# snowzurfer/raytracer-gamma

Measured on AMD Instinct MI355X. Metric: Mpixels/s (primary rays) + frame ms at WxH, depth D; PPM max-abs-diff vs CPU, higher is better.
Workload: dtype f32; 1 GPU; c3: 3840x2160, 16 spheres, 3 lights, depth 5 (RTSTACK_MAXSIZE 6), 3x3 supersampling; width=3840, height=2160, spheres=16, lights=3, depth=5, alias_factor=3, row_block=8, variant=0, parallelism=row-cyclic x1

## Files before the change

### raytracer-gamma_amd/csrc/rtg_scene_pack.h

```cpp
#pragma once

#include <math.h>
#include <string.h>

#include <algorithm>
#include <functional>
#include <thread>
#include <utility>
#include <vector>

#include "rtg.h"
#include "rtg_internal.h"
#include "rtg_trace.h"

namespace rtg {

constexpr unsigned kMaskMaxSpheres = 64;

struct PackedScene {
  std::vector<float> geom, crad2, mats, lights;
  std::vector<float> prim;
  std::vector<unsigned> smask;
  std::vector<unsigned> cone;
  std::vector<float> bvhNodes;
// ... 595 lines not shown
        cr = rc * rc;
        child = ~(int)i;
      } else {
        float mn[3] = {__builtin_inff(), __builtin_inff(), __builtin_inff()};
        float mx[3] = {-__builtin_inff(), -__builtin_inff(), -__builtin_inff()};
        for (unsigned t = a; t < b; ++t)
          for (int q = 0; q < 3; ++q) {
            mn[q] = fminf(mn[q], gb[6 * (size_t)idx[t] + q]);
            mx[q] = fmaxf(mx[q], gb[6 * (size_t)idx[t] + 3 + q]);
          }
        for (int q = 0; q < 3; ++q) {
          s[q] = mn[q];
          s[3 + q] = mx[q];
        }
        child = build(a, b, depth + 1);
      }
      float* rec = &ps->bvhNodes[(size_t)node * kBvhWords];
      for (int q = 0; q < 6; ++q) rec[6 * k + q] = s[q];
      memcpy(&rec[24 + k], &child, 4);
      rec[28 + k] = cr;
    }
    return node;
  };
  build(0, n, 0);
  if (depthOut) *depthOut = maxDepth;
  if (maxDepth > 20) {
    ps->bvhNodes.clear();
    return false;
  }
  if ((double)(ps->bvhNodes.size() / kBvhWords) * kBvhCopies * kBvhWords * 4.0 >= 0x1p32) {
    ps->bvhNodes.clear();
    return false;
  }
  {
    const std::vector<float> src = ps->bvhNodes;
    const size_t nn = src.size() / kBvhWords;
    ps->bvhNodes.assign(nn * 8 * kBvhWords, 0.f);
    for (size_t nd = 0; nd < nn; ++nd) {
      const float* in = &src[nd * kBvhWords];
      for (unsigned oct = 0; oct < 8; ++oct) {
        const double sg[3] = {(oct & 1u) ? -1.0 : 1.0, (oct & 2u) ? -1.0 : 1.0,
                              (oct & 4u) ? -1.0 : 1.0};
        int ord[4] = {0, 1, 2, 3};
        double key[4];
        int cls[4];
        for (int k = 0; k < 4; ++k) {
          int ch;
          memcpy(&ch, &in[24 + k], 4);
          key[k] = 0.0;
          cls[k] = ch > 0 ? 0 : ch < 0 ? 1 : 2;
          if (ch > 0) {
            for (int q = 0; q < 3; ++q) {
              const double lo = in[6 * k + q], hi = in[6 * k + 3 + q];
              key[k] += sg[q] * (sg[q] > 0 ? lo : hi);
            }
          } else if (ch < 0) {
            for (int q = 0; q < 3; ++q) key[k] += sg[q] * (double)in[6 * k + q];
            key[k] = key[k] * 0.5773502691896258 - (double)in[6 * k + 5];
          }
        }
        std::stable_sort(ord, ord + 4, [&](int a, int b) {
          return cls[a] != cls[b] ? cls[a] < cls[b] : key[a] < key[b];
        });
        float* out = &ps->bvhNodes[(nd * 8 + oct) * kBvhWords];
        for (int k = 0; k < 4; ++k) {
          const int j = ord[k];
          for (int q = 0; q < 6; ++q) out[6 * k + q] = in[6 * j + q];
          out[24 + k] = in[24 + j];
          out[28 + k] = in[28 + j];
        }
      }
    }
  }
  return true;
}

inline void pack_scene(const rtg_sphere* spheres, unsigned n, const rtg_light* lights,
                       unsigned m, PackedScene* ps) {
  ps->n = n;
  ps->m = m;
  ps->n4 = (n + 3u) & ~3u;
  ps->geom.assign((size_t)(ps->n4 + 4) * 20, __builtin_nanf(""));
  ps->crad2.assign(n ? 3 * (size_t)n : 1, 0.f);
  ps->mats.assign((size_t)(n + 1) * 8, 0.f);
  ps->lights.assign((size_t)(m ? m : 1) * 6, 0.f);
  ps->prim.assign((size_t)(n ? n : 1) * 4, 0.f);
  for (unsigned i = 0; i < n; ++i) {
    const rtg_sphere& s = spheres[i];
    float* g = &ps->geom[(size_t)i * 4];
    g[0] = s.pos.x; g[1] = s.pos.y; g[2] = s.pos.z;
    g[3] = s.radius * s.radius;
    float* gs = &ps->geom[(size_t)(ps->n4 + 4 + i) * 4];
    gs[0] = g[0]; gs[1] = g[1]; gs[2] = g[2];
    gs[3] = screen_r2(g[3]);
    float* gc = &ps->geom[(size_t)(2 * (ps->n4 + 4) + i) * 4];
    gc[0] = g[0]; gc[1] = g[1]; gc[2] = g[2];
    const float rc = s.radius + 1.0e-6f;
    ps->crad2[i] = rc * rc;
    gc[3] = ps->crad2[i];
    const float dx = 0.f - s.pos.x, dy = 0.f - s.pos.y, dz = 0.f - s.pos.z;
    ps->crad2[n + i] = (((dx * dx) + (dy * dy)) + (dz * dz)) - g[3];
    ps->crad2[2 * (size_t)n + i] = guard_r2(s);
    float* gf = &ps->geom[(size_t)(ps->n4 + 4) * 12 + (size_t)i * 8];
    gf[0] = g[0]; gf[1] = g[1]; gf[2] = g[2];
    gf[3] = gs[3];
    gf[4] = g[3];
    gf[5] = ps->crad2[n + i];
    gf[6] = 0.f; gf[7] = 0.f;
    prim_consts(s, &ps->prim[(size_t)i * 4]);
    float* mt = &ps->mats[(size_t)i * 8];
    mt[0] = s.material.matteColour.x; mt[1] = s.material.matteColour.y;
    mt[2] = s.material.matteColour.z; mt[3] = s.material.glossColour.x;
    mt[4] = s.material.glossColour.y; mt[5] = s.material.glossColour.z;
    mt[6] = s.material.opacity; mt[7] = s.material.refractiveIndex;
  }
  ps->mats[(size_t)n * 8 + 7] = 1.00f;
  shadow_masks(spheres, n, lights, m, &ps->smask);
  if (!ps->smask.empty()) cone_masks(spheres, n, &ps->cone);
  else ps->cone.clear();
  if (build_bvh(spheres, n, ps)) {
    sphere_lists(spheres, n, lights, m, ps);
  }
  for (unsigned l = 0; l < m; ++l) {
    float* p = &ps->lights[(size_t)l * 6];
    p[0] = lights[l].pos.x; p[1] = lights[l].pos.y; p[2] = lights[l].pos.z;
    p[3] = lights[l].col.x; p[4] = lights[l].col.y; p[5] = lights[l].col.z;
  }
}

inline int make_camera(unsigned W, unsigned H, float zoom, float aa, Camera* cam) {
  if (W == 0 || H == 0) {
    rtg_set_error("empty frame %ux%u", W, H);
    return RTG_ERR_INVALID;
  }
  if (!(aa <= 256.f)) {
    rtg_set_error("aliasFactor %g out of range", (double)aa);
    return RTG_ERR_INVALID;
  }
  cam->xs = 16.f / ((float)W);
  cam->ys = 12.f / ((float)H);
  cam->asp = 16.f / 12.f;
  cam->st = cam->xs / aa;
  const float tot = aa * aa;
  cam->inv = 1.f / tot;
  cam->halfW = W * 0.5f;
  cam->halfH = H * 0.5f;
  cam->zoom = zoom;
  int k = 0;
  while ((float)k < aa) ++k;
  cam->nAA = k;
  return RTG_OK;
}

}
```

### raytracer-gamma_amd/csrc/rtg_trace.h

```cpp
#pragma once

#include <string.h>

#include <stdint.h>
#include <math.h>

#include <type_traits>

#if defined(__HIPCC__)
#include <hip/hip_runtime.h>
#define RTG_HD __host__ __device__ __forceinline__
#else
#define RTG_HD inline
#endif

namespace rtg {

struct V3 { float x, y, z; };

RTG_HD V3 v3(float a, float b, float c) { V3 r; r.x = a; r.y = b; r.z = c; return r; }
RTG_HD V3 vadd(V3 a, V3 b) { return v3(a.x + b.x, a.y + b.y, a.z + b.z); }
RTG_HD V3 vsub(V3 a, V3 b) { return v3(a.x - b.x, a.y - b.y, a.z - b.z); }
RTG_HD V3 vmul(V3 a, V3 b) { return v3(a.x * b.x, a.y * b.y, a.z * b.z); }
RTG_HD V3 vsmul(float k, V3 b) { return v3(k * b.x, k * b.y, k * b.z); }
// ... 57 lines not shown
    no_speculate();
    if (!rcp_fast_range(b)) y = 1.f / b;
  }
  return y;
}
RTG_HD float cull_rsq(float x) {
#if defined(__HIP_DEVICE_COMPILE__)
  return __builtin_amdgcn_rsqf(x);
#else
  return 1.0f / sqrtf(x);
#endif
}
RTG_HD float rtg_sqrtf(float x) { return sqrt_rn(x); }
RTG_HD float rcp_sqrt_rn(float x) {
  float y = rcp_fast(sqrt_fast(x));
  if (any_lane(!sqrt_fast_range(x))) {
    no_speculate();
    if (!sqrt_fast_range(x)) y = 1.f / sqrtf(x);
  }
  return y;
}
RTG_HD V3 vnorm(V3 v) { float l = rcp_sqrt_rn(vdot(v, v)); return vsmul(l, v); }
RTG_HD bool significant(V3 c) { return (c.x >= 0.001f) || (c.y >= 0.001f) || (c.z >= 0.001f); }

struct Camera {
  float xs, ys, asp, st, inv, halfW, halfH, zoom;
  int nAA;
};

struct Mat { V3 matte, gloss; float opacity, refr; };

enum : int { kFusePrim = 1, kFuseCone = 2, kFuseShadow = 4, kFuseEnter = 8 };

enum : int { kCntSamples = 0, kCntPrimQ, kCntPrimSel, kCntPrimCand, kCntEnterQ, kCntEnterOK,
             kCntFullQ, kCntFullCand, kCntShadowQ, kCntShadowSel, kCntShadowCand,
             kCntContainMasked, kCntContainSel, kCntContainFull, kCntRefraction, kCntReflPush,
             kCntBvhNodeTests, kCntBvhSphereTests, kCntConeQ, kCntConeSel,
             kCntBvhShadowQ, kCntBvhShadowNodeTests, kCntBvhShadowSphereTests,
             kUQuery,
             kUPrimIter,
             kUPrimExact,
             kUSelIter,
             kUSelExact,
             kUShdIter,
             kUShdExact,
             kUEnterHead,
             kUEnterIter,
             kUEnterExact,
             kUFullGroup,
             kUFullExact,
             kUBvhNode,
             kUBvhSlot,
             kUBvhExact,
             kUContIter,
             kUCont4,
             kUContBvhNode,
             kUCone,
             kUMaskIter,
             kUNode,
             kUShade,
             kULight,
             kUShadow,
             kULit,
             kURefr,
             kURefrLeaf,
             kUPush,
             kUDescend,
             kUUnwind,
             kUSample,
             kUBvhPass,
             kUCapIter,
             kUOvIter,
             kUDiagShdSame,
             kUDiagEnterAll,
             kUDiagEnterSame,
             kUDiagContSame,
             kULightDir,
             kUDiagInsig,
             kUDiagInsigAll,
             kUWave,
             kUQueryHead,
             kUDiagShdEmpty,
             kUDiagConeEmpty,
             kCntSlots };
enum : int { kProbeClosest = 0, kProbeShadow = 1, kProbeRefraction = 2, kProbeTotal = 3,
             kProbeMatte = 4, kProbePush = 5, kProbeUnwind = 6, kProbeShade = 7,
             kProbeSlots = 8 };

struct FrameC {
  float cx, cy, cz;
  unsigned meta;
};
struct FrameR { V3 ro, rd, rI; };

template <int NF>
struct LocalFrames {
  FrameC f[NF];
  RTG_HD FrameC get(int lv) const { return f[lv]; }
  RTG_HD void set(int lv, const FrameC& v) { f[lv] = v; }
};

struct Frame {
  V3 colour;
  V3 ro, rd, rI;
  int rm;
  int flags;
};

struct RayQ {
  V3 o, d;
  float a4, den, y;
  float ap;
  bool fast;
  bool slow;
};

RTG_HD RayQ query_head(V3 o, V3 d, float& a) {
  RayQ q{};
  q.o = o;
  q.d = d;
  a = vdot(d, d);
  q.a4 = 4.0f * a;
  return q;
}
RTG_HD void query_rest(RayQ& q, float a) {
  q.den = 2.0f * a;
  q.ap = a * (1.0f - 0x1p-16f);
  q.fast = (q.den >= 0x1p-60f) && (q.den <= 0x1p60f);
  q.slow = any_lane(!q.fast);
  q.y = rcp_fast(q.den);
}

RTG_HD RayQ make_query(V3 o, V3 d) {
  float a;
  RayQ q = query_head(o, d, a);
  query_rest(q, a);
  return q;
}

RTG_HD float quot(float x, const RayQ& q) {
  const float q0 = x * q.y;
  const float r0 = fmaf(-q0, q.den, x);
  const float q1 = fmaf(r0, q.y, q0);
  const float r1 = fmaf(-q1, q.den, x);
  float r = fmaf(r1, q.y, q1);
  if (q.slow) {
    no_speculate();
    if (!q.fast) r = x / q.den;
  }
  return r;
}

template <bool kFast>
RTG_HD float quot_k(float x, const RayQ& q) {
  if constexpr (kFast) {
    const float q0 = x * q.y;
    const float r0 = fmaf(-q0, q.den, x);
    const float q1 = fmaf(r0, q.y, q0);
    const float r1 = fmaf(-q1, q.den, x);
    return fmaf(r1, q.y, q1);
  } else {
    return quot(x, q);
  }
}

#ifndef RTG_NOROOT_K
// ... 295 lines not shown
            blk = blocked_cap_lanes(sc, P, dir, gap, l, hit, cell, hc, hr2, full);
          }
          if (sc.any(full))
            if (full) blk = query_blocked<2>(sc, P, dir, gap);
        }
      } else {
        blk = query_blocked<Q>(sc, P, dir, gap);
      }
      sc.probe_end(kProbeShadow);
      if (!blk) {
        sc.count(kULit, 1);
        const float intensity = incidence / gap;
        sum = vadd(sum, vsmul(intensity, Lcol));
        if constexpr (RP::kOn) rp.lit(l);
      }
    }
  }
  return sum;
}

RTG_HD double sqrt_d_unit(double y) {
#if defined(__HIP_DEVICE_COMPILE__)
  const double g = __builtin_amdgcn_rsq(y);
  double s = y * g;
  double h = g * 0.5;
  const double r = fma(-h, s, 0.5);
  s = fma(s, r, s);
  h = fma(h, r, h);
  double d = fma(-s, s, y);
  s = fma(d, h, s);
  d = fma(-s, s, y);
  s = fma(d, h, s);
  return y == 0.0 ? 0.0 : s;
#else
  return sqrt(y);
#endif
}
RTG_HD double div_d_fresnel(double a, double b, bool fast) {
#if defined(__HIP_DEVICE_COMPILE__)
  double y = __builtin_amdgcn_rcp(b);
  double e = fma(-b, y, 1.0);
  y = fma(y, e, y);
  e = fma(-b, y, 1.0);
  y = fma(y, e, y);
  const double q = a * y;
  const double r = fma(-b, q, a);
  double d = fma(r, y, q);
  if (any_lane(!fast)) {
    no_speculate();
    if (!fast) d = a / b;
  }
  return d;
#else
  (void)fast;
  return a / b;
#endif
}

template <bool kCL = false>
RTG_HD float polarised_reflection(float n1, float n2, float cosA1, float cosA2) {
  const float left = n1 * cosA1;
  const float right = n2 * cosA2;
  if constexpr (kCL) {
    const float num = left - right;
    float den = left + right;
    den *= den;
    if (den < 1.0e-6f) return 1.f;
    float refl = (num * num) / den;
    if (refl > 1.f) refl = 1.f;
    return refl;
  }
  const double num = (double)(left - right);
  double den = (double)(left + right);
  den *= den;
  const bool tiny = den < (double)1.0e-6f;
  const bool fast = fabsf(left) <= 0x1p100f && fabsf(right) <= 0x1p100f;
  float refl = (float)div_d_fresnel(num * num, den, fast || tiny);
  if (refl > 1.f) refl = 1.f;
  return tiny ? 1.f : refl;
}

template <bool kCL = false, class Scene>
RTG_HD int refraction(const Scene& sc, V3 D, V3 P, V3 N, float nSrc, bool wantRay,
                      V3& dirOut, float& R, int hit = -1, bool guardOK = false) {
  float cosA1 = vdot(D, N);
  float sinA1 = 0.f;
  if (cosA1 <= -1.0f) { cosA1 = -1.f; sinA1 = 0.f; }
  else if (cosA1 >= 1.f) { cosA1 = 1.f; sinA1 = 0.f; }
  else sinA1 = (float)sqrt_d_unit(1.0 - (double)(cosA1 * cosA1));

  const V3 testPt = vadd(vsmul(0.01f, D), P);
  int tgt;
  float nTgt;
  if (hit >= 0 && sc.has_smask()) {
    const bool ok = guardOK && vdot(D, D) <= kContainDirMax * kContainDirMax;
    const uint64_t cu = sc.contain_union(hit, ok);
    sc.count(kCntContainMasked, 1);
    sc.count(kCntContainSel, __builtin_popcountll(cu));
    tgt = primary_container_sel(sc, testPt, cu, nTgt);
    if (tgt < 0) tgt = (int)sc.n;
  } else {
    bool full = true;
    tgt = -1;
    if (hit >= 0 && sc.has_lists() &&
        sc.all(guardOK && vdot(D, D) <= kContainDirMax * kContainDirMax)) {
      if (sc.all(sc.first_lane_i(hit) == hit)) sc.count(kUDiagContSame, 1);
      tgt = container_lanes(sc, testPt, hit, nTgt, full);
    }
    if (sc.any(full)) {
      if (full) {
        sc.count(kCntContainFull, 1);
        tgt = primary_container(sc, testPt);
        nTgt = sc.refr(tgt < 0 ? (int)sc.n : tgt);
      }
    }
    if (tgt < 0) tgt = (int)sc.n;
  }
  const float ratio = nSrc / nTgt;
  const float sinA2 = ratio * sinA1;

  if (wantRay) {
    const float qb = 2.f * cosA1;
    const float qc = 1.f - rcp_rn(ratio * ratio);
    const float rad = (qb * qb) - ((4.f * 1.f) * qc);
    float r0, r1;
    int ns;
    if (fabsf(rad) < 0.001f) {
      r0 = -qb / (2.f * 1.f);
      r1 = 0.f;
      ns = 1;
    } else {
      const float root = rtg_sqrtf(rad);
      const float den = 2.0f * 1.f;
      r0 = (-qb + root) / den;
      r1 = (-qb - root) / den;
      ns = 2;
    }
    float maxAlign = (float)-0.1;
    V3 dir = v3(0.f, 0.f, 0.f);
    {
      V3 cur = vadd(D, vsmul(r0, N));
      float al = vdot(D, cur);
      if (al > maxAlign) { maxAlign = al; dir = cur; }
    }
    if (ns == 2) {
      V3 cur = vadd(D, vsmul(r1, N));
      float al = vdot(D, cur);
      if (al > maxAlign) { maxAlign = al; dir = cur; }
    }
    dirOut = dir;
  }
  float cosA2 = rtg_sqrtf(1.f - (sinA2 * sinA2));
  if (cosA1 < 0.f) cosA2 = -cosA2;
  const float Rs = polarised_reflection<kCL>(nSrc, nTgt, cosA1, cosA2);
  const float Rp = polarised_reflection<kCL>(nSrc, nTgt, cosA2, cosA1);
  R = (Rs + Rp) * 0.5f;
  return tgt;
}

template <bool kNT>
RTG_HD void store_frame_r(FrameR& dst, const FrameR& r) {
#if defined(__HIP_DEVICE_COMPILE__)
  if constexpr (kNT) {
    __builtin_nontemporal_store(r.ro.x, &dst.ro.x);
    __builtin_nontemporal_store(r.ro.y, &dst.ro.y);
    __builtin_nontemporal_store(r.ro.z, &dst.ro.z);
    __builtin_nontemporal_store(r.rd.x, &dst.rd.x);
    __builtin_nontemporal_store(r.rd.y, &dst.rd.y);
    __builtin_nontemporal_store(r.rd.z, &dst.rd.z);
    __builtin_nontemporal_store(r.rI.x, &dst.rI.x);
    __builtin_nontemporal_store(r.rI.y, &dst.rI.y);
    __builtin_nontemporal_store(r.rI.z, &dst.rI.z);
    return;
  }
#endif
  dst = r;
}
template <bool kNT>
RTG_HD FrameR load_frame_r(const FrameR& src) {
#if defined(__HIP_DEVICE_COMPILE__)
  if constexpr (kNT) {
    FrameR r;
    r.ro = v3(__builtin_nontemporal_load(&src.ro.x), __builtin_nontemporal_load(&src.ro.y),
              __builtin_nontemporal_load(&src.ro.z));
    r.rd = v3(__builtin_nontemporal_load(&src.rd.x), __builtin_nontemporal_load(&src.rd.y),
              __builtin_nontemporal_load(&src.rd.z));
    r.rI = v3(__builtin_nontemporal_load(&src.rI.x), __builtin_nontemporal_load(&src.rI.y),
              __builtin_nontemporal_load(&src.rI.z));
    return r;
  }
#endif
  return src;
}

template <int S, int Q, bool kCL = false, class RP = NoRayPath, class Scene, class FStore>
RTG_HD V3 trace_sample(const Scene& sc, V3 dir0, FStore&& fc, bool usePrim = false,
                       uint64_t primSel = ~0ull, V3 o0 = V3{0.f, 0.f, 0.f},
                       const RP& rp = RP()) {
  static_assert(!RP::kOn || Q == 2, "a caller's rays run the Q == 2 shading path");
  constexpr int NF = (S > 1) ? (S - 1) : 1;
  FrameR fr[NF];
  int sp = 0;
  V3 ret = v3(0.f, 0.f, 0.f);
  V3 o = o0, d = dir0, I = v3(1.f, 1.f, 1.f);
  int rm = (int)sc.n;
  int enterH = -1;
  int originH = -1;
  for (;;) {
    float t;
    sc.count(kUNode, 1);
    sc.count(kUDiagInsig, significant(I) ? 0 : 1);
    if (sc.all(!significant(I))) sc.count(kUDiagInsigAll, 1);
    sc.probe_begin(kProbeClosest);
    int hit = -1;
    bool full = false;
    if constexpr (RP::kOn) {
      sc.count(kCntFullQ, 1);
      hit = rp.closest(sc, o, d, t);
    } else if (usePrim) {
      sc.count(kCntPrimQ, 1);
      sc.count(kCntPrimSel, __builtin_popcountll(primSel));
      hit = closest_hit_sel(sc, o, d, t, primSel);
      usePrim = false;
    } else if (Q == 4 && sc.has_smask() && sc.all(enterH >= 0)) {
      bool ok;
      sc.count(kUQuery, 1);
      hit = closest_enter(sc, make_query(o, d), enterH, t, ok);
      sc.count(kCntEnterQ, 1);
      sc.count(kCntEnterOK, ok ? 1 : 0);
      if (!sc.all(ok)) {
        sc.count(kCntFullQ, 1);
        hit = query_closest<2>(sc, o, d, t);
      }
    } else if (Q == 4 && sc.has_cone() && sc.all(originH >= 0)) {
      sc.count(kUCone, 1);
      const V3 dh = vsmul(cull_rsq(vdot(d, d)), d);
      const V3 U = sc.first_lane(dh);
      const float cu = vdot(dh, U);
      const int tier = sc.all(cu >= kConeCos[0]) ? 0 : sc.all(cu >= kConeCos[1]) ? 1 : -1;
      if (tier >= 0) {
// ... 6 lines not shown
          const V3 co = sc.sphere_guard(originH, r2o, g2o);
          const V3 e = vsub(q.o, co);
          if (no_root(q, 2.0f * vdot(q.d, e), vdot(e, e) - r2o)) skip = originH;
          const int h0 = sc.first_lane_i(originH);
          if (sc.all(skip == h0)) cm &= ~(1ull << h0);
        }
        sc.count(kCntConeQ, 1);
        sc.count(kCntConeSel, __builtin_popcountll(cm));
        hit = closest_sel_lazy(sc, q, qa, cm, t, skip);
      } else {
        sc.count(kCntFullQ, 1);
        hit = query_closest<2>(sc, o, d, t);
      }
    } else if (Q == 4 && sc.has_lists() && sc.any(enterH >= 0)) {
      if (sc.all(enterH >= 0) && sc.all(sc.first_lane_i(enterH) == enterH))
        sc.count(kUDiagEnterSame, 1);
      const RayQ q = make_query(o, d);
      sc.count(kUQuery, 1);
      bool todo = enterH >= 0, done = false;
      hit = -1;
      t = 1000.f;
      for (int k = 0; k < kListWalks && sc.any(todo); ++k) {
        const int h0 = sc.lane_with(enterH, todo);
        if (todo && enterH == h0) {
          bool ok;
          const int hh = closest_enter_list(sc, q, sc.first_lane_i(h0), t, ok);
          if (sc.all(ok)) {
            hit = hh;
            done = true;
          }
          todo = false;
        }
      }
      full = !done;
    } else if (!sc.has_bvh()) {
      sc.count(kCntFullQ, 1);
      hit = query_closest<Q == 4 ? 2 : Q>(sc, o, d, t);
    } else {
      if (sc.all(enterH >= 0)) sc.count(kUDiagEnterAll, 1);
      full = true;
    }
    if (sc.any(full)) {
      if (full) {
        sc.count(kCntFullQ, 1);
        hit = query_closest<Q == 4 ? 2 : Q>(sc, o, d, t);
      }
    }
    enterH = -1;
    originH = -1;
    sc.probe_end(kProbeClosest);
    sc.probe_begin(kProbeShade);
    if (hit < 0) {
      ret = vmul(I, sc.mat(rm).matte);
    } else if (significant(I)) {
      sc.count(kUShade, 1);
      V3 c;
      float g2, r2h;
      Mat mh;
      sc.hit_data(hit, c, g2, r2h, mh);
      const V3 P = vadd(o, vsmul(t, d));
      const V3 N = vnorm(vsub(P, c));
      const float op = mh.opacity;
      const float tr = 1.f - op;
      V3 colour = v3(0.f, 0.f, 0.f);
      bool guardOK = false;
      unsigned cell = kCapFull;
      if constexpr (Q == 4) {
        const V3 e = vsub(P, c);
        guardOK = vdot(e, e) <= g2;
        if (sc.has_lists() && guardOK) cell = cap_cell(e, r2h);
      }
      if (op > 0.f) {
        V3 tmp = vmul(I, mh.matte);
        tmp = vsmul(op, tmp);
        sc.probe_begin(kProbeMatte);
        const V3 mc = matte_light<Q, RP>(sc, P, N, hit, guardOK, cell, c, r2h, rp);
        sc.probe_end(kProbeMatte);
        tmp = vmul(mc, tmp);
        colour = vadd(tmp, colour);
      }
      if (tr > 0.f) {
        const bool leaf = (sp >= S - 1);
        const Mat mr = sc.mat(rm);
        V3 cdir;
        float R;
        sc.probe_begin(kProbeRefraction);
        sc.count(kCntRefraction, 1);
        sc.count(leaf ? kURefrLeaf : kURefr, 1);
        const int tgt = Q == 4 ? refraction<kCL>(sc, d, P, N, mr.refr, !leaf, cdir, R, hit, guardOK)
                               : refraction<kCL>(sc, d, P, N, mr.refr, !leaf, cdir, R);
        sc.probe_end(kProbeRefraction);
        const float prod = tr * R;
        V3 rc = vsmul(prod, v3(1.f, 1.f, 1.f));
        rc = vadd(rc, vsmul(mr.opacity, mh.gloss));
        rc = vmul(I, rc);
        const bool sigR = significant(rc);
        if (!leaf) {
          sc.probe_begin(kProbePush);
          const int lv = sp < NF ? sp : NF - 1;
          FrameC f;
          f.cx = colour.x; f.cy = colour.y; f.cz = colour.z;
          const bool origin = sc.has_cone() && guardOK;
          const bool inside = Q == 4 && origin && vdot(d, N) > 0.f;
          f.meta = ((unsigned)rm << 10) | (inside ? 0x200u : 0u) |
                   ((unsigned)(origin ? hit + 1 : 0) << 2) | (sigR ? 2u : 0u);
          if constexpr (Q == 4 && IsBvhScene<Scene>::value) {
            const bool in = sc.n < 2048u && guardOK && vdot(d, N) > 0.f;
            if (sc.n < 2048u)
              f.meta = ((unsigned)rm << 21) | ((unsigned)(in ? hit + 1 : 0) << 10) |
                       (in ? 0x200u : 0u) | (sigR ? 2u : 0u);
          }
          fc.set(lv, f);
          if (sigR) {
            sc.count(kCntReflPush, 1);
            sc.count(kUPush, 1);
            const float perp = 2.f * vdot(d, N);
            const V3 rd = vnorm(vsub(d, vsmul(perp, N)));
            FrameR r;
            r.rd = rd;
            r.ro = vadd(P, vsmul(0.01f, rd));
            r.rI = rc;
            store_frame_r<IsBvhScene<Scene>::value>(fr[lv], r);
          }
          sc.count(kUDescend, 1);
          ++sp;
          ret = colour;
          if (Q == 4 && vdot(d, N) < 0.f) enterH = hit;
          if (Q == 4 && guardOK && sc.has_cone()) originH = hit;
          I = vsmul((1.f - R), vsmul(tr, I));
          o = P;
          d = cdir;
          rm = tgt;
          sc.probe_end(kProbePush);
          sc.probe_end(kProbeShade);
          continue;
        }
        const V3 c1 = vadd(colour, colour);
        ret = (sigR && !kCL) ? vadd(c1, c1) : c1;
      } else {
        ret = colour;
      }
    }
    sc.probe_end(kProbeShade);

    sc.probe_begin(kProbeUnwind);
    bool descend = false;
    while (sp > 0) {
      sc.count(kUUnwind, 1);
      const int lv = sp - 1 < NF ? sp - 1 : NF - 1;
      FrameC f = fc.get(lv);
      const V3 fcol = vadd(ret, v3(f.cx, f.cy, f.cz));
      ret = fcol;
      if ((f.meta & 3u) == 2u) {
        f.cx = fcol.x; f.cy = fcol.y; f.cz = fcol.z;
        f.meta = (f.meta & ~3u) | 1u;
        fc.set(lv, f);
        const FrameR r = load_frame_r<IsBvhScene<Scene>::value>(fr[lv]);
        o = r.ro; d = r.rd; I = r.rI; rm = (int)(f.meta >> 10);
        originH = (int)((f.meta >> 2) & 0x7Fu) - 1;
        if (Q == 4 && (f.meta & 0x200u)) enterH = originH;
        if constexpr (Q == 4 && IsBvhScene<Scene>::value) {
          if (sc.n < 2048u) {
            rm = (int)(f.meta >> 21);
            originH = -1;
            enterH = (f.meta & 0x200u) ? (int)((f.meta >> 10) & 0x7FFu) - 1 : -1;
          }
        }
        if constexpr (kCL) ret = v3(0.f, 0.f, 0.f);
        descend = true;
        break;
      }
      --sp;
    }
    sc.probe_end(kProbeUnwind);
    if (!descend) return ret;
  }
}

template <class Scene>
// ... 1343 lines not shown
```

### raytracer-gamma_amd/rtg_amd/__init__.py

```python
from __future__ import annotations

import ctypes
import os
import sys

import numpy as np

try:
    import torch
except Exception:
    torch = None

_HERE = os.path.dirname(os.path.abspath(__file__))
LIB_PATH = os.environ.get("RTG_LIB") or os.path.join(os.path.dirname(_HERE), "librtg.so")

VEC_DTYPE = np.dtype([("x", "<f4"), ("y", "<f4"), ("z", "<f4")])
MATERIAL_DTYPE = np.dtype([("matteColour", "<f4", 3), ("glossColour", "<f4", 3),
                           ("opacity", "<f4"), ("refractiveIndex", "<f4")])
SPHERE_DTYPE = np.dtype([("pos", "<f4", 3), ("radius", "<f4"), ("material", MATERIAL_DTYPE)])
LIGHT_DTYPE = np.dtype([("pos", "<f4", 3), ("col", "<f4", 3)])
assert VEC_DTYPE.itemsize == 12 and MATERIAL_DTYPE.itemsize == 32
assert SPHERE_DTYPE.itemsize == 48 and LIGHT_DTYPE.itemsize == 24
GBUF_DTYPE = np.dtype([("id", "<i4"), ("t", "<f4"), ("hits", "<u4"), ("sample", "<u4"),
                       ("normal", "<f4", 3), ("idSum", "<u4")])
assert GBUF_DTYPE.itemsize == 32
RAY_DTYPE = np.dtype([("origin", "<f4", 3), ("dir", "<f4", 3)])
SEGMENT_DTYPE = np.dtype([("a", "<f4", 3), ("b", "<f4", 3)])
HIT_DTYPE = np.dtype([("id", "<i4"), ("t", "<f4"), ("point", "<f4", 3), ("normal", "<f4", 3)])
assert RAY_DTYPE.itemsize == 24 and SEGMENT_DTYPE.itemsize == 24 and HIT_DTYPE.itemsize == 32
CAMERA_DTYPE = np.dtype([("eye", "<f4", 3), ("right", "<f4", 3), ("up", "<f4", 3),
                         ("back", "<f4", 3)])
assert CAMERA_DTYPE.itemsize == 48
AO_PARAMS_DTYPE = np.dtype([("samples", "<u4"), ("radius", "<f4"), ("bias", "<f4"),
                            ("seed", "<u4"), ("flags", "<u4")])
assert AO_PARAMS_DTYPE.itemsize == 20
AO_MAX_SAMPLES, AO_MAX_DIRS, AO_JITTER = 1024, 65536, 1
FOLD_PARAMS_DTYPE = np.dtype([("viewsPerGroup", "<u4"), ("weights", "<u4"), ("flags", "<u4")])
assert FOLD_PARAMS_DTYPE.itemsize == 12
FOLD_MAX_WEIGHTS, FOLD_SKIP_NONFINITE = 16, 1

RTG_OK = 0
ERRORS = {-1: "invalid argument", -2: "HIP error", -3: "out of memory",
          -4: "no such device", -5: "I/O error"}

EXPORTED = [
    "rtg_last_error", "rtg_abi_version", "rtg_device_count", "rtg_device_info",
    "rtg_render", "rtg_context_create", "rtg_context_destroy", "rtg_context_set_scene",
    "rtg_shard_rows", "rtg_shard_global_row", "rtg_render_device", "rtg_render_rows_device",
    "rtg_render_rows", "rtg_set_launch_opts", "rtg_diag_read", "rtg_diag_timeline", "rtg_diag_counts",
    "rtg_diag_group_list",
    "rtg_context_scene_stats",
    "rtg_max_colour", "rtg_max_colour_device", "rtg_ppm_bytes", "rtg_ppm_bytes_device",
    "rtg_save_ppm", "rtg_make_material", "rtg_scene_generate", "rtg_assemble_shards_device",
    "rtg_render_multi", "rtg_scene_load", "rtg_scene_save", "rtg_context_set_semantics",
    "rtg_multi_create", "rtg_multi_set_scene", "rtg_multi_render", "rtg_multi_destroy",
    "rtg_multi_set_gather", "rtg_place_shard_device",
    "rtg_gbuffer_device", "rtg_gbuffer", "rtg_gbuffer_host",
    "rtg_intersect_device", "rtg_intersect", "rtg_intersect_host",
    "rtg_visible_device", "rtg_visible", "rtg_visible_host",
    "rtg_raytrace_device", "rtg_raytrace", "rtg_raytrace_host",
    "rtg_ray_order_scratch", "rtg_ray_order_device", "rtg_ray_order_host",
    "rtg_intersect_indexed_device", "rtg_visible_indexed_device", "rtg_raytrace_indexed_device",
    "rtg_camera_identity", "rtg_camera_look_at", "rtg_camera_sample_count",
    "rtg_camera_rays_host", "rtg_camera_rays_device",
    "rtg_render_camera_device", "rtg_render_camera", "rtg_render_camera_host",
    "rtg_render_views_device", "rtg_render_views", "rtg_render_views_host", "rtg_camera_cube",
    "rtg_views_fold_scratch", "rtg_views_fold_host", "rtg_views_fold_device",
    "rtg_render_views_fold_device", "rtg_render_views_fold", "rtg_render_views_fold_host",
    "rtg_cube_sh_weights",
    "rtg_ao_directions", "rtg_ao_segments_host", "rtg_ao_segments_device", "rtg_ao_device",
    "rtg_ao", "rtg_ao_host",
    "rtg_matte_device", "rtg_matte", "rtg_matte_host",
    "rtg_contains_device", "rtg_contains", "rtg_contains_host",
]


UNIT_NAMES = [
    "samples", "primQ", "primSel", "primCand", "enterQ", "enterOK", "fullQ", "fullCand",
    "shadowQ", "shadowSel", "shadowCand", "containMasked", "containSel", "containFull",
    "refraction", "reflPush", "bvhNodeTests", "bvhSphereTests", "coneQ", "coneSel",
    "bvhShadowQ", "bvhShadowNodeTests", "bvhShadowSphereTests",
    "U.query", "U.primIter", "U.primExact", "U.selIter", "U.selExact", "U.shdIter",
    "U.shdExact", "U.enterHead", "U.enterIter", "U.enterExact", "U.fullGroup", "U.fullExact",
    "U.bvhNode", "U.bvhSlot", "U.bvhExact", "U.contIter", "U.cont4", "U.contBvhNode", "U.cone",
    "U.maskIter", "U.node", "U.shade", "U.light", "U.shadow", "U.lit", "U.refr", "U.refrLeaf",
    "U.push", "U.descend", "U.unwind", "U.sample", "U.bvhPass",
    "U.capIter", "U.ovIter", "D.shdSame", "D.enterAll", "D.enterSame", "D.contSame",
    "U.lightDir", "D.insig", "D.insigAll", "U.wave",
    "U.queryHead", "D.shdEmpty", "D.coneEmpty",
]


class RtgError(RuntimeError):
    pass


_lib = None


def lib() -> ctypes.CDLL:
    global _lib
    if _lib is None:
        if not os.path.exists(LIB_PATH):
            raise RtgError(f"librtg.so not built at {LIB_PATH}; run __graft_entry__.build()")
        L = ctypes.CDLL(LIB_PATH)
        vp, u, i, f, sz = ctypes.c_void_p, ctypes.c_uint, ctypes.c_int, ctypes.c_float, ctypes.c_size_t
        L.rtg_last_error.restype = ctypes.c_char_p
        L.rtg_abi_version.restype = i
        L.rtg_device_count.argtypes = [ctypes.POINTER(i)]
        L.rtg_device_info.argtypes = [i, ctypes.c_char_p, sz]
        L.rtg_render.argtypes = [i, vp, u, vp, u, u, u, f, f, i, vp]
        L.rtg_context_create.argtypes = [i, ctypes.POINTER(vp)]
        L.rtg_context_destroy.argtypes = [vp]
        L.rtg_context_set_scene.argtypes = [vp, vp, u, vp, u]
        L.rtg_shard_rows.argtypes = [u, u, u, u, ctypes.POINTER(u)]
        L.rtg_shard_global_row.argtypes = [u, u, u, u]
        L.rtg_shard_global_row.restype = u
        L.rtg_render_device.argtypes = [vp, u, u, f, f, i, u, u, u, vp, vp]
        L.rtg_render_rows_device.argtypes = [vp, u, u, f, f, i, vp, u, vp, vp]
        L.rtg_render_rows.argtypes = [i, vp, u, vp, u, u, u, f, f, i, vp, u, vp]
        L.rtg_set_launch_opts.argtypes = [vp, vp]
        L.rtg_context_set_semantics.argtypes = [vp, i]
        L.rtg_diag_read.argtypes = [vp, vp, i]
        L.rtg_diag_timeline.argtypes = [vp, vp, sz, vp]
        if hasattr(L, "rtg_diag_group_list"):
            L.rtg_diag_group_list.argtypes = [vp, vp, vp, vp, vp, sz, vp]
        for name, at in (("rtg_diag_counts", [vp, vp, i, i]),
                         ("rtg_context_scene_stats", [vp, vp]),
                         ("rtg_multi_set_gather", [vp, i]),
                         ("rtg_place_shard_device", [vp, vp, u, u, u, u, u, vp, vp])):
            try:
                getattr(L, name).argtypes = at
            except AttributeError:
                if not os.environ.get("RTG_LIB"):
                    raise
        L.rtg_max_colour.argtypes = [vp, sz]
        L.rtg_max_colour.restype = f
        L.rtg_max_colour_device.argtypes = [vp, vp, sz, vp, vp]
        L.rtg_ppm_bytes.argtypes = [vp, sz, f, vp]
        L.rtg_ppm_bytes.restype = None
        L.rtg_ppm_bytes_device.argtypes = [vp, vp, sz, vp, vp, vp]
        L.rtg_assemble_shards_device.argtypes = [vp, vp, u, u, u, u, u, vp, vp]
        L.rtg_render_multi.argtypes = [vp, i, vp, u, vp, u, u, u, f, f, i, u, vp, vp]
        L.rtg_multi_create.argtypes = [vp, i, ctypes.POINTER(vp)]
        L.rtg_multi_set_scene.argtypes = [vp, vp, u, vp, u]
        L.rtg_multi_render.argtypes = [vp, u, u, f, f, i, u, vp, vp]
        L.rtg_multi_destroy.argtypes = [vp]
        L.rtg_gbuffer_device.argtypes = [vp, u, u, f, f, u, u, u, vp, vp]
        L.rtg_gbuffer.argtypes = [i, vp, u, u, u, f, f, vp]
        L.rtg_gbuffer_host.argtypes = [vp, u, u, u, f, f, vp, i]
        for q in ("intersect", "visible"):
            getattr(L, f"rtg_{q}_device").argtypes = [vp, vp, sz, vp, vp]
            getattr(L, f"rtg_{q}").argtypes = [i, vp, u, vp, sz, vp]
            getattr(L, f"rtg_{q}_host").argtypes = [vp, u, vp, sz, vp, i, i]
        L.rtg_raytrace_device.argtypes = [vp, vp, sz, i, vp, vp]
        L.rtg_raytrace.argtypes = [i, vp, u, vp, u, vp, sz, i, vp]
        L.rtg_raytrace_host.argtypes = [vp, u, vp, u, vp, sz, i, i, vp, i, i]
        L.rtg_ray_order_scratch.argtypes = [sz, ctypes.POINTER(sz)]
        L.rtg_ray_order_device.argtypes = [vp, vp, sz, i, vp, vp, vp, sz, vp]
        L.rtg_ray_order_host.argtypes = [vp, u, vp, sz, i, vp, vp, i]
        L.rtg_intersect_indexed_device.argtypes = [vp, vp, vp, sz, vp, vp]
        L.rtg_visible_indexed_device.argtypes = [vp, vp, vp, sz, vp, vp]
        L.rtg_raytrace_indexed_device.argtypes = [vp, vp, vp, sz, i, vp, vp]
        L.rtg_camera_identity.argtypes = [vp]
        L.rtg_camera_identity.restype = None
        L.rtg_camera_look_at.argtypes = [vp, vp, vp, vp]
        L.rtg_camera_sample_count.argtypes = [f, ctypes.POINTER(u)]
        L.rtg_camera_rays_host.argtypes = [vp, u, u, f, f, vp, i]
        L.rtg_camera_rays_device.argtypes = [vp, vp, u, u, f, f, vp, vp]
        L.rtg_render_camera_device.argtypes = [vp, vp, u, u, f, f, i, vp, vp]
        L.rtg_render_camera.argtypes = [i, vp, u, vp, u, vp, u, u, f, f, i, vp]
        L.rtg_render_camera_host.argtypes = [vp, u, vp, u, vp, u, u, f, f, i, i, vp, i, i]
# ... 914 lines not shown
```

### raytracer-gamma_amd/rtg_amd/work.py

```python
from __future__ import annotations

UNIT_COST = {
    "U.query": 16,
    "U.queryHead": 6,
    "U.primIter": 10,
    "U.primExact": 36,
    "U.selIter": 12,
    "U.selExact": 55,
    "U.shdIter": 13,
    "U.shdExact": 62,
    "U.enterHead": 77,
    "U.enterIter": 22,
    "U.enterExact": 39,
    "U.fullGroup": 48,
    "U.fullExact": 59,
    "U.bvhNode": 2,
    "U.bvhSlot": 20,
    "U.bvhExact": 60,
    "U.contIter": 13,
    "U.cont4": 43,
    "U.contBvhNode": 48,
    "U.cone": 17,
    "U.maskIter": 4,
    "U.node": 12,
    "U.shade": 55,
    "U.light": 12,
    "U.lightDir": 30,
    "U.shadow": 3,
    "U.lit": 16,
    "U.refr": 245,
    "U.refrLeaf": 185,
    "U.push": 48,
    "U.descend": 28,
    "U.unwind": 12,
    "U.capIter": 13,
    "U.ovIter": 13,
    "U.sample": 80,
    "U.wave": 20,
}

FIT_RECORD = "profiles/r06/calib_units/fit.json"
UNIT_COST_SOURCE = dict(UNIT_COST)
UNIT_COST.update({
    "U.query": 19.97,
    "U.primIter": 11.58,
    "U.primExact": 48.38,
    "U.selIter": 11.43,
    "U.selExact": 55.98,
    "U.shdIter": 13.54,
    "U.shdExact": 57.52,
    "U.enterHead": 81.57,
    "U.enterIter": 21.97,
    "U.enterExact": 39.09,
    "U.fullGroup": 50.98,
    "U.fullExact": 81.25,
    "U.bvhNode": 2.0,
    "U.bvhSlot": 20.39,
    "U.bvhExact": 59.4,
    "U.contIter": 12.8,
    "U.contBvhNode": 47.32,
    "U.cone": 16.8,
    "U.maskIter": 4.02,
    "U.node": 13.37,
    "U.shade": 81.94,
    "U.light": 12.84,
    "U.lightDir": 35.96,
    "U.shadow": 3.06,
    "U.lit": 17.88,
    "U.refr": 216.57,
    "U.refrLeaf": 270.71,
    "U.push": 50.08,
    "U.descend": 27.69,
    "U.unwind": 11.92,
    "U.capIter": 10.3,
    "U.ovIter": 11.19,
    "U.sample": 136.0,
    "U.wave": 26.08,
})

VALU_PEAK_TOPS = 256 * 4 * 32 * 2.4e9 / 1e12


def executed_work(names, waves, lanes=None):
    units = {}
    slots = 0
    for k, nm in enumerate(names):
        if nm not in UNIT_COST:
            continue
        w = int(waves[k])
        s = w * UNIT_COST[nm]
        slots += s
        units[nm] = {"waves": w, "slots": s}
        if lanes is not None:
            units[nm]["lanes"] = int(lanes[k])
            units[nm]["lane_util"] = round(int(lanes[k]) / (64.0 * w), 3) if w else None
    return {"valu_slots": slots, "lane_ops": 64 * slots, "units": units}
```

Before: 6608 Mpixels/s.

## Skip leaf refraction work when result cannot be significant

```diff
diff --git a/raytracer-gamma_amd/csrc/rtg_scene_pack.h b/raytracer-gamma_amd/csrc/rtg_scene_pack.h
--- a/raytracer-gamma_amd/csrc/rtg_scene_pack.h
+++ b/raytracer-gamma_amd/csrc/rtg_scene_pack.h
@@ -701,7 +701,7 @@
   ps->n4 = (n + 3u) & ~3u;
   ps->geom.assign((size_t)(ps->n4 + 4) * 20, __builtin_nanf(""));
   ps->crad2.assign(n ? 3 * (size_t)n : 1, 0.f);
-  ps->mats.assign((size_t)(n + 1) * 8, 0.f);
+  ps->mats.assign((size_t)(n + 2) * 8, 0.f);
   ps->lights.assign((size_t)(m ? m : 1) * 6, 0.f);
   ps->prim.assign((size_t)(n ? n : 1) * 4, 0.f);
   for (unsigned i = 0; i < n; ++i) {
@@ -734,6 +734,13 @@
     mt[6] = s.material.opacity; mt[7] = s.material.refractiveIndex;
   }
   ps->mats[(size_t)n * 8 + 7] = 1.00f;
+  float nMin = 1.00f;
+  for (unsigned i = 0; i < n; ++i) {
+    const float ri = spheres[i].material.refractiveIndex;
+    if (!(ri > 0.f && ri < __builtin_inff())) nMin = -__builtin_inff();
+    else if (ri < nMin) nMin = ri;
+  }
+  ps->mats[(size_t)(n + 1) * 8 + 7] = nMin;
   shadow_masks(spheres, n, lights, m, &ps->smask);
   if (!ps->smask.empty()) cone_masks(spheres, n, &ps->cone);
   else ps->cone.clear();
diff --git a/raytracer-gamma_amd/csrc/rtg_trace.h b/raytracer-gamma_amd/csrc/rtg_trace.h
--- a/raytracer-gamma_amd/csrc/rtg_trace.h
+++ b/raytracer-gamma_amd/csrc/rtg_trace.h
@@ -163,6 +163,13 @@
              kUQueryHead,
              kUDiagShdEmpty,
              kUDiagConeEmpty,
+             kURefrLeafFull,
+             kURefrLeafTir,
+             kUDiagLeafSkip,
+             kUDiagLeafZero,
+             kUDiagLeafCL,
+             kUDiagLeafFalse,
+             kUDiagLeafFree,
              kCntSlots };
 enum : int { kProbeClosest = 0, kProbeShadow = 1, kProbeRefraction = 2, kProbeTotal = 3,
              kProbeMatte = 4, kProbePush = 5, kProbeUnwind = 6, kProbeShade = 7,
@@ -624,7 +631,8 @@
 
 template <bool kCL = false, class Scene>
 RTG_HD int refraction(const Scene& sc, V3 D, V3 P, V3 N, float nSrc, bool wantRay,
-                      V3& dirOut, float& R, int hit = -1, bool guardOK = false) {
+                      V3& dirOut, float& R, int hit = -1, bool guardOK = false,
+                      bool wantR = true) {
   float cosA1 = vdot(D, N);
   float sinA1 = 0.f;
   if (cosA1 <= -1.0f) { cosA1 = -1.f; sinA1 = 0.f; }
@@ -694,10 +702,93 @@
   }
   float cosA2 = rtg_sqrtf(1.f - (sinA2 * sinA2));
   if (cosA1 < 0.f) cosA2 = -cosA2;
-  const float Rs = polarised_reflection<kCL>(nSrc, nTgt, cosA1, cosA2);
-  const float Rp = polarised_reflection<kCL>(nSrc, nTgt, cosA2, cosA1);
-  R = (Rs + Rp) * 0.5f;
+  R = cosA2 * cosA2;
+  if (wantR) {
+    const float Rs = polarised_reflection<kCL>(nSrc, nTgt, cosA1, cosA2);
+    const float Rp = polarised_reflection<kCL>(nSrc, nTgt, cosA2, cosA1);
+    R = (Rs + Rp) * 0.5f;
+  }
   return tgt;
+}
+
+enum : int { kLeafFull = 0, kLeafTir = 1, kLeafFree = 2, kLeafZero = 3, kLeafCL = 4, kLeafFalse = 5 };
+#ifndef RTG_LEAF_RULES
+#define RTG_LEAF_RULES 0x3E
+#endif
+template <class S, class = void>
+struct LeafRules : std::integral_constant<int, RTG_LEAF_RULES> {};
+template <class S>
+struct LeafRules<S, std::void_t<decltype(S::kLeafRules)>> : std::integral_constant<int, S::kLeafRules> {};
+
+template <bool kCL, int kRules>
+RTG_HD int leaf_rule(V3 colour, V3 I, float tr, V3 k, float nSrc, V3 D, V3 N, float nMin) {
+  constexpr bool r1 = kRules >> kLeafZero & 1, r2 = (kRules >> kLeafCL & 1) && kCL,
+                 r3 = kRules >> kLeafFalse & 1, r4f = kRules >> kLeafFree & 1,
+                 r4t = kRules >> kLeafTir & 1;
+  if (r2 && !r1) return kLeafCL;
+  const bool zero = r1 && colour.x == 0.f && colour.y == 0.f && colour.z == 0.f;
+  if (r2) return zero ? kLeafZero : kLeafCL;
+  if (!r3 && !r4f && !r4t) return zero ? kLeafZero : kLeafFull;
+  float sum, top, both;
+  {
+    const float a = I.x * k.x, b = I.x * (tr + k.x);
+    sum = fabsf(a) + fabsf(b);
+    top = fmaxf(a, b);
+    both = fminf(a, b);
+  }
+  {
+    const float a = I.y * k.y, b = I.y * (tr + k.y);
+    sum = (sum + fabsf(a)) + fabsf(b);
+    top = fmaxf(top, fmaxf(a, b));
+    both = fmaxf(both, fminf(a, b));
+  }
+  {
+    const float a = I.z * k.z, b = I.z * (tr + k.z);
+    sum = (sum + fabsf(a)) + fabsf(b);
+    top = fmaxf(top, fmaxf(a, b));
+    both = fmaxf(both, fminf(a, b));
+  }
+  if (zero) return kLeafZero;
+  if (!(sum < __builtin_inff())) return kLeafFull;
+  if (!(top >= 0.001f)) return r3 ? kLeafFalse : kLeafFull;
+  if (!(both >= 0.001f)) return kLeafFull;
+  const float cosA1 = vdot(D, N);
+  if (r4f && nSrc <= nMin && cosA1 == cosA1) return kLeafFree;
+  return (r4t && nMin > 0.f) ? kLeafTir : kLeafFull;
+}
+
+template <bool kCL, bool kHit, class Scene>
+RTG_HD bool refract_node(const Scene& sc, bool leaf, V3 colour, V3 I, float tr, V3 kg, float nSrc,
+                         V3 d, V3 P, V3 N, int hit, bool guardOK, V3& cdir, float& R, int& tgt,
+                         V3& rc) {
+  sc.count(kCntRefraction, 1);
+  sc.count(leaf ? kURefrLeaf : kURefr, 1);
+  int rule = kLeafFull;
+  if (leaf) {
+    rule = leaf_rule<kCL, LeafRules<Scene>::value>(colour, I, tr, kg, nSrc, d, N,
+                                                   sc.refr((int)sc.n + 1));
+    if (rule == kLeafFull) sc.count(kURefrLeafFull, 1);
+    else if (rule == kLeafTir) sc.count(kURefrLeafTir, 1);
+    else if (rule == kLeafZero) sc.count(kUDiagLeafZero, 1);
+    else if (rule == kLeafCL) sc.count(kUDiagLeafCL, 1);
+    else if (rule == kLeafFalse) sc.count(kUDiagLeafFalse, 1);
+    else sc.count(kUDiagLeafFree, 1);
+  }
+  if (!sc.any(rule <= kLeafTir)) sc.count(kUDiagLeafSkip, 1);
+  bool sigR = rule == kLeafFree;
+  if (sc.any(rule <= kLeafTir)) {
+    if (rule <= kLeafTir) {
+      const bool fres = rule == kLeafFull;
+      tgt = kHit ? refraction<kCL>(sc, d, P, N, nSrc, !leaf, cdir, R, hit, guardOK, fres)
+                 : refraction<kCL>(sc, d, P, N, nSrc, !leaf, cdir, R, -1, false, fres);
+      const float prod = tr * R;
+      rc = vsmul(prod, v3(1.f, 1.f, 1.f));
+      rc = vadd(rc, kg);
+      rc = vmul(I, rc);
+      sigR = significant(rc);
+    }
+  }
+  return sigR;
 }
 
 template <bool kNT>
@@ -870,19 +961,14 @@
       if (tr > 0.f) {
         const bool leaf = (sp >= S - 1);
         const Mat mr = sc.mat(rm);
-        V3 cdir;
-        float R;
+        V3 cdir = v3(0.f, 0.f, 0.f), rc = cdir;
+        float R = 0.f;
+        int tgt = rm;
         sc.probe_begin(kProbeRefraction);
-        sc.count(kCntRefraction, 1);
-        sc.count(leaf ? kURefrLeaf : kURefr, 1);
-        const int tgt = Q == 4 ? refraction<kCL>(sc, d, P, N, mr.refr, !leaf, cdir, R, hit, guardOK)
-                               : refraction<kCL>(sc, d, P, N, mr.refr, !leaf, cdir, R);
+        const bool sigR = refract_node<kCL, Q == 4>(sc, leaf, colour, I, tr,
+                                                    vsmul(mr.opacity, mh.gloss), mr.refr, d, P, N,
+                                                    hit, guardOK, cdir, R, tgt, rc);
         sc.probe_end(kProbeRefraction);
-        const float prod = tr * R;
-        V3 rc = vsmul(prod, v3(1.f, 1.f, 1.f));
-        rc = vadd(rc, vsmul(mr.opacity, mh.gloss));
-        rc = vmul(I, rc);
-        const bool sigR = significant(rc);
         if (!leaf) {
           sc.probe_begin(kProbePush);
           const int lv = sp < NF ? sp : NF - 1;
diff --git a/raytracer-gamma_amd/rtg_amd/__init__.py b/raytracer-gamma_amd/rtg_amd/__init__.py
--- a/raytracer-gamma_amd/rtg_amd/__init__.py
+++ b/raytracer-gamma_amd/rtg_amd/__init__.py
@@ -88,6 +88,8 @@
     "U.capIter", "U.ovIter", "D.shdSame", "D.enterAll", "D.enterSame", "D.contSame",
     "U.lightDir", "D.insig", "D.insigAll", "U.wave",
     "U.queryHead", "D.shdEmpty", "D.coneEmpty",
+    "U.refrLeafFull", "U.refrLeafTir", "D.leafSkip", "D.leafZero", "D.leafCL", "D.leafFalse",
+    "D.leafFree",
 ]
 
 
diff --git a/raytracer-gamma_amd/rtg_amd/work.py b/raytracer-gamma_amd/rtg_amd/work.py
--- a/raytracer-gamma_amd/rtg_amd/work.py
+++ b/raytracer-gamma_amd/rtg_amd/work.py
@@ -29,7 +29,9 @@
     "U.shadow": 3,
     "U.lit": 16,
     "U.refr": 245,
-    "U.refrLeaf": 185,
+    "U.refrLeaf": 44,
+    "U.refrLeafFull": 182,
+    "U.refrLeafTir": 87,
     "U.push": 48,
     "U.descend": 28,
     "U.unwind": 12,
@@ -68,7 +70,7 @@
     "U.shadow": 3.06,
     "U.lit": 17.88,
     "U.refr": 216.57,
-    "U.refrLeaf": 270.71,
+    "U.refrLeafFull": 270.71,
     "U.push": 50.08,
     "U.descend": 27.69,
     "U.unwind": 11.92,
```

Measured after the change: 6604 Mpixels/s. No clear change (-0.1%).
